# BatsResearch/menghini-neurips23-code

Hardware: AMD Instinct MI355X
Metric: images/sec CLIP ViT-B/16 encode+prompt-step (higher is better)
Workload: dtype f16

## Files before the change

menghini-neurips23-code_amd/csrc/attention_split.hip:

```cpp
#include <math.h>

#include "common.h"

__device__ __forceinline__ int vt_index_fwd_s(int key, int d) { return vt_index(key, ((d >> 2) & 3) * 16 + (d >> 4) * 4 + (d & 3)); }

__device__ __forceinline__ void split8(const f32x4 a, const f32x4 b, half8& hi, half8& lo) {
    half4 h0, l0, h1, l1;
    split_f16x4(a, h0, l0);
    split_f16x4(b, h1, l1);
    hi = (half8){h0[0], h0[1], h0[2], h0[3], h1[0], h1[1], h1[2], h1[3]};
    lo = (half8){l0[0], l0[1], l0[2], l0[3], l1[0], l1[1], l1[2], l1[3]};
}

template <int KVC, bool CAUSAL, int NW>
__global__ __launch_bounds__(NW * 64) void attn_fwd_split_kernel(const float* __restrict__ qkv, half_t* __restrict__ out, int S, int H) {
    constexpr int SP = KVC * 32;
    constexpr float LOG2E = 1.4426950408889634f;
    constexpr float INV = 1.0f / (float)GRIP_SPLIT_LO_SCALE;
    extern __shared__ __attribute__((aligned(16))) char smem[];
    half_t* Kh = (half_t*)smem;
    half_t* Kl = Kh + SP * 64;
    half_t* Vh = Kl + SP * 64;
    half_t* Vl = Vh + SP * 64;

    const int tid = threadIdx.x, lane = tid & 63, wave = tid >> 6;
    const int D = H * 64;
    const int b = blockIdx.x / H, h = blockIdx.x - b * H;
    const size_t ld = (size_t)3 * D;
    const float* base = qkv + (size_t)b * S * ld + h * 64;
    const int li = lane & 15, lg = lane >> 4;
    const int n_qt = (S + 15) >> 4;

    for (int idx = tid; idx < SP * 8; idx += NW * 64) {
        const int row = idx >> 3, chunk = idx & 7;
        f32x4 a = {0.f, 0.f, 0.f, 0.f}, c = {0.f, 0.f, 0.f, 0.f};
        if (row < S) {
            const f32x4* p = (const f32x4*)(base + (size_t)row * ld + D + chunk * 8);
            a = p[0];
            c = p[1];
        }
        half8 hi, lo;
        split8(a, c, hi, lo);
        const int o = row * 64 + ((chunk ^ (row & 7)) * 8);
        *(half8*)(Kh + o) = hi;
        *(half8*)(Kl + o) = lo;
    }
    for (int idx = tid; idx < ((SP / 2 + 31) / 32) * 256; idx += NW * 64) {
        const int lane_rp = idx & 31, chunk = ((idx >> 5) & 1) + 2 * ((idx >> 6) & 3), rblk = idx >> 8;
        const int r0 = 2 * (rblk * 32 + lane_rp);
        if (r0 >= SP) continue;
        f32x4 z = {0.f, 0.f, 0.f, 0.f};
        f32x4 a0 = z, a1 = z, b0 = z, b1 = z;
        if (r0 < S) { const f32x4* p = (const f32x4*)(base + (size_t)r0 * ld + 2 * D + chunk * 8); a0 = p[0]; a1 = p[1]; }
        if (r0 + 1 < S) { const f32x4* p = (const f32x4*)(base + (size_t)(r0 + 1) * ld + 2 * D + chunk * 8); b0 = p[0]; b1 = p[1]; }
        half8 h0, l0, h1, l1;
        split8(a0, a1, h0, l0);
        split8(b0, b1, h1, l1);
#pragma unroll
        for (int j = 0; j < 8; ++j) {
            const int o = vt_index_fwd_s(r0, chunk * 8 + j);
            *(half2v*)(Vh + o) = (half2v){h0[j], h1[j]};
            *(half2v*)(Vl + o) = (half2v){l0[j], l1[j]};
        }
    }
    __syncthreads();

    for (int qt = wave; qt < n_qt; qt += NW) {
        asm volatile("" ::: "memory");
        const int qrow = qt * 16 + li;
        const int qr = qrow < S ? qrow : S - 1;
        half8 qh[2], ql[2];
#pragma unroll
        for (int kk = 0; kk < 2; ++kk) {
            const f32x4* p = (const f32x4*)(base + (size_t)qr * ld + (kk * 4 + lg) * 8);
            split8(p[0] * 0.125f, p[1] * 0.125f, qh[kk], ql[kk]);
        }
        f32x4 sc[2 * KVC];
        float m = -INFINITY;
#pragma unroll
        for (int t = 0; t < 2 * KVC; ++t) {
            f32x4 acc = {0.f, 0.f, 0.f, 0.f}, cor = {0.f, 0.f, 0.f, 0.f};
#pragma unroll
            for (int kk = 0; kk < 2; ++kk) {
                const int o = (t * 16 + li) * 64 + (((kk * 4 + lg) ^ (lane & 7)) * 8);
                const half8 kh = *(const half8*)(Kh + o), kl = *(const half8*)(Kl + o);
                acc = __builtin_amdgcn_mfma_f32_16x16x32_f16(kh, qh[kk], acc, 0, 0, 0);
                cor = __builtin_amdgcn_mfma_f32_16x16x32_f16(kl, qh[kk], cor, 0, 0, 0);
                cor = __builtin_amdgcn_mfma_f32_16x16x32_f16(kh, ql[kk], cor, 0, 0, 0);
            }
            acc += cor * INV;
            if (CAUSAL || t >= 2 * (KVC - 1)) {
#pragma unroll
                for (int r = 0; r < 4; ++r) {
                    const int kv = t * 16 + lg * 4 + r;
                    if (kv >= S || (CAUSAL && kv > qrow)) acc[r] = -INFINITY;
                }
            }
            m = fmaxf(fmaxf(fmaxf(m, acc[0]), fmaxf(acc[1], acc[2])), acc[3]);
            sc[t] = acc;
        }
        m = fmaxf(m, __shfl_xor(m, 16));
        m = fmaxf(m, __shfl_xor(m, 32));
        const float m2 = m * LOG2E;
#pragma unroll
        for (int t = 0; t < 2 * KVC; ++t)
#pragma unroll
            for (int r = 0; r < 4; ++r) sc[t][r] = __builtin_amdgcn_exp2f(__builtin_fmaf(sc[t][r], LOG2E, -m2));

        const half8 ones = {1, 1, 1, 1, 1, 1, 1, 1};
        f32x4 sum_h = {0.f, 0.f, 0.f, 0.f}, sum_l = {0.f, 0.f, 0.f, 0.f};
        f32x4 o[4], oc[4];
#pragma unroll
        for (int nf = 0; nf < 4; ++nf) { o[nf] = (f32x4){0.f, 0.f, 0.f, 0.f}; oc[nf] = (f32x4){0.f, 0.f, 0.f, 0.f}; }
#pragma unroll
        for (int c = 0; c < KVC; ++c) {
            half8 ph, pl;
            split8(sc[2 * c], sc[2 * c + 1], ph, pl);
#pragma unroll
            for (int nf = 0; nf < 4; ++nf) {
                const int vo = (c * 4 + nf) * 512 + (lg * 16 + (li ^ lg)) * 8;
                const half8 vh = *(const half8*)(Vh + vo), vl = *(const half8*)(Vl + vo);
                o[nf] = __builtin_amdgcn_mfma_f32_16x16x32_f16(vh, ph, o[nf], 0, 0, 0);
                oc[nf] = __builtin_amdgcn_mfma_f32_16x16x32_f16(vl, ph, oc[nf], 0, 0, 0);
                oc[nf] = __builtin_amdgcn_mfma_f32_16x16x32_f16(vh, pl, oc[nf], 0, 0, 0);
            }
            sum_h = __builtin_amdgcn_mfma_f32_16x16x32_f16(ones, ph, sum_h, 0, 0, 0);
            sum_l = __builtin_amdgcn_mfma_f32_16x16x32_f16(ones, pl, sum_l, 0, 0, 0);
        }
        if (qrow < S) {
            const float inv = 1.0f / (sum_h[0] + sum_l[0] * INV);
            half_t* orow = out + (size_t)((size_t)b * S + qrow) * 2 * D;
            const int col = h * 64 + lg * 16;
            half_t* op = orow + (col >> 5) * 64 + (col & 31);
            half8 hi0, lo0, hi1, lo1;
            split8((o[0] + oc[0] * INV) * inv, (o[1] + oc[1] * INV) * inv, hi0, lo0);
            split8((o[2] + oc[2] * INV) * inv, (o[3] + oc[3] * INV) * inv, hi1, lo1);
            *(half8*)op = hi0;
            *(half8*)(op + 8) = hi1;
            *(half8*)(op + 32) = lo0;
            *(half8*)(op + 40) = lo1;
        }
    }
}

bool attention_split_supported(int S) { return S >= 1 && S <= 320; }

int launch_attention_fwd_split(const float* qkv, void* out, int B, int S, int H, int causal, hipStream_t s) {
    GRIP_REQUIRE(attention_split_supported(S) && B >= 1 && H >= 1, "attention_split: bad shape B=%d S=%d H=%d (S <= 320)", B, S, H);
    const int kvc = (S + 31) / 32;
    const size_t lds = (size_t)4 * kvc * 32 * 64 * sizeof(half_t);
#define GRIP_ATT_CASE(K)                                                                                                                     \
    case K: {                                                                                                                                \
        static bool configured = false;                                                                                                      \
        if (!configured) {                                                                                                                   \
            GRIP_CHECK_HIP(hipFuncSetAttribute((const void*)attn_fwd_split_kernel<K, false, (K >= 4 ? 8 : 4)>, hipFuncAttributeMaxDynamicSharedMemorySize, (int)lds)); \
            GRIP_CHECK_HIP(hipFuncSetAttribute((const void*)attn_fwd_split_kernel<K, true, (K >= 4 ? 8 : 4)>, hipFuncAttributeMaxDynamicSharedMemorySize, (int)lds));  \
            configured = true;                                                                                                               \
        }                                                                                                                                    \
        if (causal) hipLaunchKernelGGL((attn_fwd_split_kernel<K, true, (K >= 4 ? 8 : 4)>), dim3(B * H), dim3((K >= 4 ? 8 : 4) * 64), lds, s, qkv, (half_t*)out, S, H); \
        else hipLaunchKernelGGL((attn_fwd_split_kernel<K, false, (K >= 4 ? 8 : 4)>), dim3(B * H), dim3((K >= 4 ? 8 : 4) * 64), lds, s, qkv, (half_t*)out, S, H);       \
    } break;
    switch (kvc) {
        GRIP_ATT_CASE(1) GRIP_ATT_CASE(2) GRIP_ATT_CASE(3) GRIP_ATT_CASE(4) GRIP_ATT_CASE(5)
        GRIP_ATT_CASE(6) GRIP_ATT_CASE(7) GRIP_ATT_CASE(8) GRIP_ATT_CASE(9) GRIP_ATT_CASE(10)
        default: GRIP_REQUIRE(false, "attention_split: S = %d out of range", S);
    }
#undef GRIP_ATT_CASE
    GRIP_CHECK_HIP(hipGetLastError());
    return GRIP_OK;
}
```

Baseline: 20960.

## Software-pipeline split attention: batch K/V staging loads, prefetch Q, double-buffer LDS reads

K and V staging now issues all global loads into registers before converting and writing to LDS, and the next Q tile is prefetched during the current tile's compute. The QK^T and PV inner loops double-buffer LDS fragment reads around MFMA groups using sched_barrier, and the last score tile is skipped when S fits in fewer tiles. Launch bounds now carry a per-config minimum-waves hint. The intent is to hide global and LDS latency behind MFMA work, at the cost of higher register pressure and more complex scheduling.

```diff
diff --git a/menghini-neurips23-code_amd/csrc/attention_split.hip b/menghini-neurips23-code_amd/csrc/attention_split.hip
--- a/menghini-neurips23-code_amd/csrc/attention_split.hip
+++ b/menghini-neurips23-code_amd/csrc/attention_split.hip
@@ -1,4 +1,6 @@
 #include <math.h>
+
+#include <type_traits>
 
 #include "common.h"
 
@@ -12,9 +14,14 @@
     lo = (half8){l0[0], l0[1], l0[2], l0[3], l1[0], l1[1], l1[2], l1[3]};
 }
 
+constexpr int split_attn_min_waves(int kvc, bool causal, int nw) {
+    return nw == 8 ? ((kvc <= 5 && !causal) ? 4 : 2) : (causal && kvc == 3) ? 3 : 4;
+}
+
 template <int KVC, bool CAUSAL, int NW>
-__global__ __launch_bounds__(NW * 64) void attn_fwd_split_kernel(const float* __restrict__ qkv, half_t* __restrict__ out, int S, int H) {
+__global__ __launch_bounds__(NW * 64, split_attn_min_waves(KVC, CAUSAL, NW)) void attn_fwd_split_kernel(const float* __restrict__ qkv, half_t* __restrict__ out, int S, int H) {
     constexpr int SP = KVC * 32;
+    constexpr int NTH = NW * 64;
     constexpr float LOG2E = 1.4426950408889634f;
     constexpr float INV = 1.0f / (float)GRIP_SPLIT_LO_SCALE;
     extern __shared__ __attribute__((aligned(16))) char smem[];
@@ -31,74 +38,157 @@
     const int li = lane & 15, lg = lane >> 4;
     const int n_qt = (S + 15) >> 4;
 
-    for (int idx = tid; idx < SP * 8; idx += NW * 64) {
-        const int row = idx >> 3, chunk = idx & 7;
-        f32x4 a = {0.f, 0.f, 0.f, 0.f}, c = {0.f, 0.f, 0.f, 0.f};
-        if (row < S) {
-            const f32x4* p = (const f32x4*)(base + (size_t)row * ld + D + chunk * 8);
-            a = p[0];
-            c = p[1];
-        }
-        half8 hi, lo;
-        split8(a, c, hi, lo);
-        const int o = row * 64 + ((chunk ^ (row & 7)) * 8);
-        *(half8*)(Kh + o) = hi;
-        *(half8*)(Kl + o) = lo;
-    }
-    for (int idx = tid; idx < ((SP / 2 + 31) / 32) * 256; idx += NW * 64) {
+    auto q_load = [&](int qt, f32x4 (&q)[4]) {
+        const int qrow = qt * 16 + li;
+        const int qr = qrow < S ? qrow : S - 1;
+#pragma unroll
+        for (int kk = 0; kk < 2; ++kk) {
+            const f32x4* p = (const f32x4*)(base + (size_t)qr * ld + (kk * 4 + lg) * 8);
+            q[2 * kk] = p[0];
+            q[2 * kk + 1] = p[1];
+        }
+    };
+
+    constexpr int KT = (SP * 8 + NTH - 1) / NTH;
+    constexpr int VT = (((SP / 2 + 31) / 32) * 256 + NTH - 1) / NTH;
+    const f32x4 z4 = {0.f, 0.f, 0.f, 0.f};
+    f32x4 kr[KT][2], vr[VT][4], qn[4];
+#pragma unroll
+    for (int i = 0; i < KT; ++i) {
+        const int idx = tid + i * NTH, row = idx >> 3, chunk = idx & 7;
+        const f32x4* p = (const f32x4*)(base + (size_t)(row < S ? row : S - 1) * ld + D + chunk * 8);
+        kr[i][0] = p[0];
+        kr[i][1] = p[1];
+    }
+#pragma unroll
+    for (int i = 0; i < VT; ++i) {
+        const int idx = tid + i * NTH;
         const int lane_rp = idx & 31, chunk = ((idx >> 5) & 1) + 2 * ((idx >> 6) & 3), rblk = idx >> 8;
         const int r0 = 2 * (rblk * 32 + lane_rp);
-        if (r0 >= SP) continue;
-        f32x4 z = {0.f, 0.f, 0.f, 0.f};
-        f32x4 a0 = z, a1 = z, b0 = z, b1 = z;
-        if (r0 < S) { const f32x4* p = (const f32x4*)(base + (size_t)r0 * ld + 2 * D + chunk * 8); a0 = p[0]; a1 = p[1]; }
-        if (r0 + 1 < S) { const f32x4* p = (const f32x4*)(base + (size_t)(r0 + 1) * ld + 2 * D + chunk * 8); b0 = p[0]; b1 = p[1]; }
+        const f32x4* p0 = (const f32x4*)(base + (size_t)(r0 < S ? r0 : S - 1) * ld + 2 * D + chunk * 8);
+        const f32x4* p1 = (const f32x4*)(base + (size_t)(r0 + 1 < S ? r0 + 1 : S - 1) * ld + 2 * D + chunk * 8);
+        vr[i][0] = p0[0]; vr[i][1] = p0[1];
+        vr[i][2] = p1[0]; vr[i][3] = p1[1];
+    }
+    q_load(wave, qn);
+    __builtin_amdgcn_sched_barrier(0);
+#pragma unroll
+    for (int i = 0; i < KT; ++i) {
+        const int idx = tid + i * NTH, row = idx >> 3, chunk = idx & 7;
+        half8 hi, lo;
+        split8(row < S ? kr[i][0] : z4, row < S ? kr[i][1] : z4, hi, lo);
+        if (idx < SP * 8) {
+            const int o = row * 64 + ((chunk ^ (row & 7)) * 8);
+            *(half8*)(Kh + o) = hi;
+            *(half8*)(Kl + o) = lo;
+        }
+    }
+#pragma unroll
+    for (int i = 0; i < VT; ++i) {
+        const int idx = tid + i * NTH;
+        const int lane_rp = idx & 31, chunk = ((idx >> 5) & 1) + 2 * ((idx >> 6) & 3), rblk = idx >> 8;
+        const int r0 = 2 * (rblk * 32 + lane_rp);
         half8 h0, l0, h1, l1;
-        split8(a0, a1, h0, l0);
-        split8(b0, b1, h1, l1);
-#pragma unroll
-        for (int j = 0; j < 8; ++j) {
-            const int o = vt_index_fwd_s(r0, chunk * 8 + j);
-            *(half2v*)(Vh + o) = (half2v){h0[j], h1[j]};
-            *(half2v*)(Vl + o) = (half2v){l0[j], l1[j]};
+        split8(r0 < S ? vr[i][0] : z4, r0 < S ? vr[i][1] : z4, h0, l0);
+        split8(r0 + 1 < S ? vr[i][2] : z4, r0 + 1 < S ? vr[i][3] : z4, h1, l1);
+        if (r0 < SP) {
+#pragma unroll
+            for (int j = 0; j < 8; ++j) {
+                const int o = vt_index_fwd_s(r0, chunk * 8 + j);
+                *(half2v*)(Vh + o) = (half2v){h0[j], h1[j]};
+                *(half2v*)(Vl + o) = (half2v){l0[j], l1[j]};
+            }
         }
     }
     __syncthreads();
+
+    const int ko0 = li * 64 + ((lg ^ (lane & 7)) * 8), ko1 = li * 64 + (((4 + lg) ^ (lane & 7)) * 8);
+    const int vo0 = (lg * 16 + (li ^ lg)) * 8;
+    constexpr int KG = split_attn_min_waves(KVC, CAUSAL, NW) == 2 ? 2 : 1, PG = KG;
+    auto k_read = [&](int u0, int kb0, int kb1, half8 (&f)[2 * KG]) {
+#pragma unroll
+        for (int j = 0; j < KG; ++j) {
+            const int u = u0 + j, o = (u >> 1) * 1024 + ((u & 1) ? kb1 : kb0);
+            f[2 * j] = *(const half8*)(Kh + o);
+            f[2 * j + 1] = *(const half8*)(Kl + o);
+        }
+    };
+    auto v_read = [&](int g0, int vb, half8 (&f)[2 * PG]) {
+#pragma unroll
+        for (int j = 0; j < PG; ++j) {
+            f[2 * j] = *(const half8*)(Vh + (g0 + j) * 512 + vb);
+            f[2 * j + 1] = *(const half8*)(Vl + (g0 + j) * 512 + vb);
+        }
+    };
 
     for (int qt = wave; qt < n_qt; qt += NW) {
         asm volatile("" ::: "memory");
+        int kb0 = ko0, kb1 = ko1, vb = vo0;
+        asm volatile("" : "+v"(kb0), "+v"(kb1), "+v"(vb));
         const int qrow = qt * 16 + li;
-        const int qr = qrow < S ? qrow : S - 1;
         half8 qh[2], ql[2];
 #pragma unroll
-        for (int kk = 0; kk < 2; ++kk) {
-            const f32x4* p = (const f32x4*)(base + (size_t)qr * ld + (kk * 4 + lg) * 8);
-            split8(p[0] * 0.125f, p[1] * 0.125f, qh[kk], ql[kk]);
-        }
+        for (int kk = 0; kk < 2; ++kk) split8(qn[2 * kk] * 0.125f, qn[2 * kk + 1] * 0.125f, qh[kk], ql[kk]);
+        if (qt + NW < n_qt) q_load(qt + NW, qn);
         f32x4 sc[2 * KVC];
         float m = -INFINITY;
-#pragma unroll
-        for (int t = 0; t < 2 * KVC; ++t) {
-            f32x4 acc = {0.f, 0.f, 0.f, 0.f}, cor = {0.f, 0.f, 0.f, 0.f};
-#pragma unroll
-            for (int kk = 0; kk < 2; ++kk) {
-                const int o = (t * 16 + li) * 64 + (((kk * 4 + lg) ^ (lane & 7)) * 8);
-                const half8 kh = *(const half8*)(Kh + o), kl = *(const half8*)(Kl + o);
-                acc = __builtin_amdgcn_mfma_f32_16x16x32_f16(kh, qh[kk], acc, 0, 0, 0);
-                cor = __builtin_amdgcn_mfma_f32_16x16x32_f16(kl, qh[kk], cor, 0, 0, 0);
-                cor = __builtin_amdgcn_mfma_f32_16x16x32_f16(kh, ql[kk], cor, 0, 0, 0);
+        auto scores = [&](auto nt_c) {
+            constexpr int NT = decltype(nt_c)::value;
+            half8 kf[2][2 * KG];
+            f32x4 cor[2];
+            auto finish = [&](int t) {
+                f32x4 acc = sc[t];
+                acc += cor[t & 1] * INV;
+                if (CAUSAL || t >= 2 * (KVC - 1)) {
+#pragma unroll
+                    for (int r = 0; r < 4; ++r) {
+                        const int kv = t * 16 + lg * 4 + r;
+                        if (kv >= S || (CAUSAL && kv > qrow)) acc[r] = -INFINITY;
+                    }
+                }
+                m = fmaxf(fmaxf(fmaxf(m, acc[0]), fmaxf(acc[1], acc[2])), acc[3]);
+                sc[t] = acc;
+            };
+            k_read(0, kb0, kb1, kf[0]);
+#pragma unroll
+            for (int u0 = 0; u0 < 2 * NT; u0 += KG) {
+                const int t = u0 >> 1;
+                if (u0 + KG < 2 * NT) k_read(u0 + KG, kb0, kb1, kf[(u0 / KG + 1) & 1]);
+                __builtin_amdgcn_sched_barrier(0);
+                const half8(&f)[2 * KG] = kf[(u0 / KG) & 1];
+                const f32x4 z = {0.f, 0.f, 0.f, 0.f};
+                if (KG == 2) {
+                    f32x4 acc = z, c = z;
+                    acc = __builtin_amdgcn_mfma_f32_16x16x32_f16(f[0], qh[0], acc, 0, 0, 0);
+                    c = __builtin_amdgcn_mfma_f32_16x16x32_f16(f[1], qh[0], c, 0, 0, 0);
+                    acc = __builtin_amdgcn_mfma_f32_16x16x32_f16(f[2 * KG - 2], qh[1], acc, 0, 0, 0);
+                    c = __builtin_amdgcn_mfma_f32_16x16x32_f16(f[0], ql[0], c, 0, 0, 0);
+                    c = __builtin_amdgcn_mfma_f32_16x16x32_f16(f[2 * KG - 1], qh[1], c, 0, 0, 0);
+                    c = __builtin_amdgcn_mfma_f32_16x16x32_f16(f[2 * KG - 2], ql[1], c, 0, 0, 0);
+                    sc[t] = acc;
+                    cor[t & 1] = c;
+                } else {
+                    const int kk = u0 & 1;
+                    f32x4 acc = kk ? sc[t] : z, c = kk ? cor[t & 1] : z;
+                    acc = __builtin_amdgcn_mfma_f32_16x16x32_f16(f[0], qh[kk], acc, 0, 0, 0);
+                    c = __builtin_amdgcn_mfma_f32_16x16x32_f16(f[1], qh[kk], c, 0, 0, 0);
+                    c = __builtin_amdgcn_mfma_f32_16x16x32_f16(f[0], ql[kk], c, 0, 0, 0);
+                    sc[t] = acc;
+                    cor[t & 1] = c;
+                }
+                if (t > 0 && (u0 & 1) == 0) finish(t - 1);
+                __builtin_amdgcn_sched_barrier(0);
             }
-            acc += cor * INV;
-            if (CAUSAL || t >= 2 * (KVC - 1)) {
-#pragma unroll
-                for (int r = 0; r < 4; ++r) {
-                    const int kv = t * 16 + lg * 4 + r;
-                    if (kv >= S || (CAUSAL && kv > qrow)) acc[r] = -INFINITY;
-                }
-            }
-            m = fmaxf(fmaxf(fmaxf(m, acc[0]), fmaxf(acc[1], acc[2])), acc[3]);
-            sc[t] = acc;
-        }
+            finish(NT - 1);
+        };
+        if (S > (2 * KVC - 1) * 16) {
+            scores(std::integral_constant<int, 2 * KVC>{});
+        } else {
+            scores(std::integral_constant<int, 2 * KVC - 1>{});
+            sc[2 * KVC - 1] = (f32x4){-INFINITY, -INFINITY, -INFINITY, -INFINITY};
+        }
+        half8 vf[2][2 * PG];
+        v_read(0, vb, vf[0]);
         m = fmaxf(m, __shfl_xor(m, 16));
         m = fmaxf(m, __shfl_xor(m, 32));
         const float m2 = m * LOG2E;
@@ -112,20 +202,27 @@
         f32x4 o[4], oc[4];
 #pragma unroll
         for (int nf = 0; nf < 4; ++nf) { o[nf] = (f32x4){0.f, 0.f, 0.f, 0.f}; oc[nf] = (f32x4){0.f, 0.f, 0.f, 0.f}; }
-#pragma unroll
-        for (int c = 0; c < KVC; ++c) {
-            half8 ph, pl;
-            split8(sc[2 * c], sc[2 * c + 1], ph, pl);
-#pragma unroll
-            for (int nf = 0; nf < 4; ++nf) {
-                const int vo = (c * 4 + nf) * 512 + (lg * 16 + (li ^ lg)) * 8;
-                const half8 vh = *(const half8*)(Vh + vo), vl = *(const half8*)(Vl + vo);
-                o[nf] = __builtin_amdgcn_mfma_f32_16x16x32_f16(vh, ph, o[nf], 0, 0, 0);
-                oc[nf] = __builtin_amdgcn_mfma_f32_16x16x32_f16(vl, ph, oc[nf], 0, 0, 0);
-                oc[nf] = __builtin_amdgcn_mfma_f32_16x16x32_f16(vh, pl, oc[nf], 0, 0, 0);
+        half8 ph, pl, phn, pln;
+        split8(sc[0], sc[1], ph, pl);
+#pragma unroll
+        for (int g0 = 0; g0 < 4 * KVC; g0 += PG) {
+            const int c = g0 >> 2, n0 = g0 & 3;
+            if (g0 + PG < 4 * KVC) v_read(g0 + PG, vb, vf[(g0 / PG + 1) & 1]);
+            __builtin_amdgcn_sched_barrier(0);
+            const half8(&f)[2 * PG] = vf[(g0 / PG) & 1];
+#pragma unroll
+            for (int j = 0; j < PG; ++j) o[n0 + j] = __builtin_amdgcn_mfma_f32_16x16x32_f16(f[2 * j], ph, o[n0 + j], 0, 0, 0);
+#pragma unroll
+            for (int j = 0; j < PG; ++j) oc[n0 + j] = __builtin_amdgcn_mfma_f32_16x16x32_f16(f[2 * j + 1], ph, oc[n0 + j], 0, 0, 0);
+#pragma unroll
+            for (int j = 0; j < PG; ++j) oc[n0 + j] = __builtin_amdgcn_mfma_f32_16x16x32_f16(f[2 * j], pl, oc[n0 + j], 0, 0, 0);
+            if (n0 + PG == 4) {
+                if (c + 1 < KVC) split8(sc[2 * c + 2], sc[2 * c + 3], phn, pln);
+                sum_h = __builtin_amdgcn_mfma_f32_16x16x32_f16(ones, ph, sum_h, 0, 0, 0);
+                sum_l = __builtin_amdgcn_mfma_f32_16x16x32_f16(ones, pl, sum_l, 0, 0, 0);
             }
-            sum_h = __builtin_amdgcn_mfma_f32_16x16x32_f16(ones, ph, sum_h, 0, 0, 0);
-            sum_l = __builtin_amdgcn_mfma_f32_16x16x32_f16(ones, pl, sum_l, 0, 0, 0);
+            __builtin_amdgcn_sched_barrier(0);
+            if (n0 + PG == 4) { ph = phn; pl = pln; }
         }
         if (qrow < S) {
             const float inv = 1.0f / (sum_h[0] + sum_l[0] * INV);
```

Result: no change. 21020 (median of 6 runs) (+0.3%).
